# DecaYale/RNNPose

Hardware: AMD Instinct MI355X
Metric: pose-refine iters/sec (640x480, B=8, 3x8 recurrent) (higher is better)
Workload: dtype f32 (convolutions and volume build: fp16x3-split MFMA, fp32-class accuracy; LM: f64)

## Files before the change

rnnpose_amd/csrc/nhwc_ops.hip:

```cpp
#define RP_CONTRACT_LOCAL 1
#include "common.hpp"
#include "f16x3.cuh"
#include "induced.cuh"

namespace {

__global__ __launch_bounds__(256) void nchw_to_nhwc_kernel(const float* __restrict__ src, float* __restrict__ dst, int C,
                                                           int HW, int dst_cs, int dst_co) {
  __shared__ float tile[32][33];
  const int b = blockIdx.z;
  const int p0 = blockIdx.x * 32, c0 = blockIdx.y * 32;
  const int tx = threadIdx.x & 31, ty = threadIdx.x >> 5;
#pragma unroll
  for (int r = 0; r < 4; ++r) {
    const int c = c0 + ty + 8 * r, pp = p0 + tx;
    tile[ty + 8 * r][tx] = (c < C && pp < HW) ? src[(static_cast<long long>(b) * C + c) * HW + pp] : 0.f;
  }
  __syncthreads();
#pragma unroll
  for (int r = 0; r < 4; ++r) {
    const int pp = p0 + ty + 8 * r, c = c0 + tx;
    if (c < C && pp < HW) dst[(static_cast<long long>(b) * HW + pp) * dst_cs + dst_co + c] = tile[tx][ty + 8 * r];
  }
}

__global__ __launch_bounds__(256) void nhwc_to_nchw_kernel(const float* __restrict__ src, float* __restrict__ dst, int C,
                                                           int HW, int src_cs, int src_co) {
  __shared__ float tile[32][33];
  const int b = blockIdx.z;
  const int p0 = blockIdx.x * 32, c0 = blockIdx.y * 32;
  const int tx = threadIdx.x & 31, ty = threadIdx.x >> 5;
#pragma unroll
  for (int r = 0; r < 4; ++r) {
    const int pp = p0 + ty + 8 * r, c = c0 + tx;
    tile[ty + 8 * r][tx] = (c < C && pp < HW) ? src[(static_cast<long long>(b) * HW + pp) * src_cs + src_co + c] : 0.f;
  }
  __syncthreads();
#pragma unroll
  for (int r = 0; r < 4; ++r) {
    const int c = c0 + ty + 8 * r, pp = p0 + tx;
    if (c < C && pp < HW) dst[(static_cast<long long>(b) * C + c) * HW + pp] = tile[tx][ty + 8 * r];
  }
}

__global__ __launch_bounds__(256) void flow_prep_kernel(const float* __restrict__ coords1, float* __restrict__ flow4,
                                                        float* __restrict__ motion, int motion_cs, int motion_co, int h,
                                                        int w, long long total, int subtract_grid) {
  const long long t = static_cast<long long>(blockIdx.x) * blockDim.x + threadIdx.x;
  if (t >= total) return;
  const int n = h * w;
  const int b = static_cast<int>(t / n), pix = static_cast<int>(t - static_cast<long long>(b) * n);
  const int X = pix % w, Y = pix / w;
  const float fx = coords1[(static_cast<long long>(b) * 2 + 0) * n + pix] - (subtract_grid ? static_cast<float>(X) : 0.f);
  const float fy = coords1[(static_cast<long long>(b) * 2 + 1) * n + pix] - (subtract_grid ? static_cast<float>(Y) : 0.f);
  *reinterpret_cast<float4*>(flow4 + t * 4) = make_float4(fx, fy, 0.f, 0.f);
  *reinterpret_cast<float2*>(motion + t * motion_cs + motion_co) = make_float2(fx, fy);
}

__global__ __launch_bounds__(256) void conv3x3_cout2_kernel(const float* __restrict__ x, int cs, int co, int Cin,
                                                            const float* __restrict__ wgt, const float* __restrict__ bias,
                                                            const float* __restrict__ coords1, float* __restrict__ delta,
                                                            float* __restrict__ coords1_out, float* __restrict__ flow_lr,
                                                            int B, int h, int w) {
  extern __shared__ float wl[];
  const int tid = threadIdx.x;
  for (int e = tid; e < 2 * 9 * Cin; e += 256) {
    const int c = e % Cin, tap = (e / Cin) % 9, o = e / (9 * Cin);
    wl[e] = wgt[(static_cast<long long>(o) * Cin + c) * 9 + tap];
  }
  __syncthreads();
  const int lane = tid & 63, wave = tid >> 6;
  const int n = h * w;
  const long long total = static_cast<long long>(B) * n;
  for (long long p = static_cast<long long>(blockIdx.x) * 4 + wave; p < total; p += static_cast<long long>(gridDim.x) * 4) {
    const int b = static_cast<int>(p / n), pix = static_cast<int>(p - static_cast<long long>(b) * n);
    const int X = pix % w, Y = pix / w;
    float a0 = 0.f, a1 = 0.f;
    for (int c = lane * 4; c < Cin; c += 256) {
#pragma unroll
      for (int tap = 0; tap < 9; ++tap) {
        const int yy = Y + tap / 3 - 1, xx = X + tap % 3 - 1;
        if (yy < 0 || yy >= h || xx < 0 || xx >= w) continue;
        const float4 v = *reinterpret_cast<const float4*>(x + (static_cast<long long>(b) * n + yy * w + xx) * cs + co + c);
        const float4 w0 = *reinterpret_cast<const float4*>(wl + (0 * 9 + tap) * Cin + c);
        const float4 w1 = *reinterpret_cast<const float4*>(wl + (1 * 9 + tap) * Cin + c);
        a0 += v.x * w0.x + v.y * w0.y + v.z * w0.z + v.w * w0.w;
        a1 += v.x * w1.x + v.y * w1.y + v.z * w1.z + v.w * w1.w;
      }
    }
#pragma unroll
    for (int d = 32; d >= 1; d >>= 1) {
      a0 += __shfl_down(a0, d);
      a1 += __shfl_down(a1, d);
    }
    if (lane == 0) {
      const float dx = a0 + bias[0], dy = a1 + bias[1];
      *reinterpret_cast<float2*>(delta + p * 2) = make_float2(dx, dy);
      const float cx = coords1[(static_cast<long long>(b) * 2 + 0) * n + pix] + dx;
      const float cy = coords1[(static_cast<long long>(b) * 2 + 1) * n + pix] + dy;
      if (coords1_out) {
        coords1_out[(static_cast<long long>(b) * 2 + 0) * n + pix] = cx;
        coords1_out[(static_cast<long long>(b) * 2 + 1) * n + pix] = cy;
      }
      *reinterpret_cast<float2*>(flow_lr + p * 2) = make_float2(cx - static_cast<float>(X), cy - static_cast<float>(Y));
    }
  }
}

__global__ __launch_bounds__(256) void conv3x3_cout2_run4_kernel(const float* __restrict__ x, int cs, int co, int Cin,
                                                                 const float* __restrict__ wgt, const float* __restrict__ bias,
                                                                 const float* __restrict__ coords1, float* __restrict__ delta,
                                                                 float* __restrict__ coords1_out, float* __restrict__ flow_lr,
                                                                 int B, int h, int w) {
  const int lane = threadIdx.x & 63, wave = threadIdx.x >> 6;
  const int c = lane * 4;
  const bool cl = c < Cin;
  float4 w0[9], w1[9];
  {
    float t0[36], t1[36];
#pragma unroll
    for (int e = 0; e < 9; ++e) {
      const float4 z = make_float4(0.f, 0.f, 0.f, 0.f);
      const float4 q0 = cl ? *reinterpret_cast<const float4*>(wgt + (static_cast<long long>(0) * Cin + c) * 9 + e * 4) : z;
      const float4 q1 = cl ? *reinterpret_cast<const float4*>(wgt + (static_cast<long long>(1) * Cin + c) * 9 + e * 4) : z;
      t0[e * 4 + 0] = q0.x; t0[e * 4 + 1] = q0.y; t0[e * 4 + 2] = q0.z; t0[e * 4 + 3] = q0.w;
      t1[e * 4 + 0] = q1.x; t1[e * 4 + 1] = q1.y; t1[e * 4 + 2] = q1.z; t1[e * 4 + 3] = q1.w;
    }
#pragma unroll
    for (int tap = 0; tap < 9; ++tap) {
      w0[tap] = make_float4(t0[tap], t0[9 + tap], t0[18 + tap], t0[27 + tap]);
      w1[tap] = make_float4(t1[tap], t1[9 + tap], t1[18 + tap], t1[27 + tap]);
    }
  }
  const int n = h * w;
  const int runs_per_row = (w + 3) >> 2;
  const long long total_runs = static_cast<long long>(B) * h * runs_per_row;
  for (long long r = static_cast<long long>(blockIdx.x) * 4 + wave; r < total_runs; r += static_cast<long long>(gridDim.x) * 4) {
    const unsigned ru = static_cast<unsigned>(r);
    const unsigned by = ru / static_cast<unsigned>(runs_per_row);
    const int xr = static_cast<int>(ru - by * runs_per_row);
    const int b = static_cast<int>(by / static_cast<unsigned>(h)), Y = static_cast<int>(by - static_cast<unsigned>(b) * h);
    const int X0 = xr * 4;
    const int idx = ((lane >> 5) & 1) * 4 + ((lane >> 4) & 1) * 2 + ((lane >> 3) & 1);
    const int px = idx >> 1, o = idx & 1;
    const int Xw = X0 + px < w ? X0 + px : w - 1;
    const int pixw = Y * w + Xw;
    const float c1x = coords1[(static_cast<long long>(b) * 2 + 0) * n + pixw];
    const float c1y = coords1[(static_cast<long long>(b) * 2 + 1) * n + pixw];
    float4 v[3][6];
#pragma unroll
    for (int ry = 0; ry < 3; ++ry)
#pragma unroll
      for (int cx = 0; cx < 6; ++cx) {
        const int yy = Y + ry - 1, xx = X0 + cx - 1;
        const bool ok = cl && yy >= 0 && yy < h && xx >= 0 && xx < w;
        v[ry][cx] = ok ? *reinterpret_cast<const float4*>(x + (static_cast<long long>(b) * n + yy * w + xx) * cs + co + c)
                       : make_float4(0.f, 0.f, 0.f, 0.f);
      }
    float acc[8];
#pragma unroll
    for (int px = 0; px < 4; ++px) {
      float a0 = 0.f, a1 = 0.f;
#pragma unroll
      for (int ry = 0; ry < 3; ++ry)
#pragma unroll
        for (int k = 0; k < 3; ++k) {
          const float4 q = v[ry][px + k], u0 = w0[ry * 3 + k], u1 = w1[ry * 3 + k];
          a0 += q.x * u0.x + q.y * u0.y + q.z * u0.z + q.w * u0.w;
          a1 += q.x * u1.x + q.y * u1.y + q.z * u1.z + q.w * u1.w;
        }
      acc[px * 2 + 0] = a0;
      acc[px * 2 + 1] = a1;
    }
    float s4[4], s2[2], s1;
    {
      const bool up = lane & 32;
#pragma unroll
      for (int i = 0; i < 4; ++i) {
        const float keep = up ? acc[4 + i] : acc[i], give = up ? acc[i] : acc[4 + i];
        s4[i] = keep + __shfl_xor(give, 32);
      }
      const bool up2 = lane & 16;
#pragma unroll
      for (int i = 0; i < 2; ++i) {
        const float keep = up2 ? s4[2 + i] : s4[i], give = up2 ? s4[i] : s4[2 + i];
        s2[i] = keep + __shfl_xor(give, 16);
      }
      const bool up3 = lane & 8;
      const float keep = up3 ? s2[1] : s2[0], give = up3 ? s2[0] : s2[1];
      s1 = keep + __shfl_xor(give, 8);
      s1 += __shfl_xor(s1, 4);
      s1 += __shfl_xor(s1, 2);
      s1 += __shfl_xor(s1, 1);
    }
    const float other = __shfl_xor(s1, 8);
    if ((lane & 7) == 0 && o == 0 && X0 + px < w) {
      const int X = X0 + px, pix = Y * w + X;
      const long long p = static_cast<long long>(b) * n + pix;
      const float dx = s1 + bias[0], dy = other + bias[1];
      *reinterpret_cast<float2*>(delta + p * 2) = make_float2(dx, dy);
      const float cxv = c1x + dx;
      const float cyv = c1y + dy;
      if (coords1_out) {
        coords1_out[(static_cast<long long>(b) * 2 + 0) * n + pix] = cxv;
        coords1_out[(static_cast<long long>(b) * 2 + 1) * n + pix] = cyv;
      }
      *reinterpret_cast<float2*>(flow_lr + p * 2) = make_float2(cxv - static_cast<float>(X), cyv - static_cast<float>(Y));
    }
  }
}

__global__ __launch_bounds__(256) void convex_upsample_nhwc_kernel(const float* __restrict__ flow,
                                                                   const float* __restrict__ mask,
                                                                   float* __restrict__ up, int h, int w) {
  const int b = blockIdx.z, Y = blockIdx.y;
  const int X = blockIdx.x * 4 + (threadIdx.x >> 6);
  const int t = threadIdx.x & 63;
  if (X >= w) return;
  const int n = h * w;
  const float* m = mask + (static_cast<long long>(b) * n + Y * w + X) * 576 + t;
  float mv[9], mx = -INFINITY;
  float2 fv[9];
#pragma unroll
  for (int k = 0; k < 9; ++k) {
    mv[k] = m[k * 64];
    const int yy = Y + k / 3 - 1, xx = X + k % 3 - 1;
    const bool ok = yy >= 0 && yy < h && xx >= 0 && xx < w;
    fv[k] = *reinterpret_cast<const float2*>(flow + (static_cast<long long>(b) * n + (ok ? yy * w + xx : Y * w + X)) * 2);
  }
  __builtin_amdgcn_sched_barrier(0);
#pragma unroll
  for (int k = 0; k < 9; ++k) mx = fmaxf(mx, mv[k]);
  float den = 0.f;
#pragma unroll
  for (int k = 0; k < 9; ++k) {
    mv[k] = expf(mv[k] - mx);
    den += mv[k];
  }
  float ax = 0.f, ay = 0.f;
#pragma unroll
  for (int k = 0; k < 9; ++k) {
    const int yy = Y + k / 3 - 1, xx = X + k % 3 - 1;
    const float2 f = (yy >= 0 && yy < h && xx >= 0 && xx < w) ? fv[k] : make_float2(0.f, 0.f);
    const float wk = mv[k] / den;
    ax += wk * (8.f * f.x);
    ay += wk * (8.f * f.y);
  }
  const int i = t >> 3, j = t & 7;
  const long long Wf = 8LL * w, Pf = 64LL * n;
  const long long o = (8LL * Y + i) * Wf + 8 * X + j;
  up[(static_cast<long long>(b) * 2 + 0) * Pf + o] = ax;
  up[(static_cast<long long>(b) * 2 + 1) * Pf + o] = ay;
}


constexpr int IN_ROWS = 512;
__global__ __launch_bounds__(256) void instnorm_partial_kernel(const float* __restrict__ x, double* __restrict__ part,
                                                               int HW, int C) {
  __shared__ double s1[256], s2[256];
  const int b = blockIdx.y, chunk = blockIdx.x, nchunk = gridDim.x;
  const int tid = threadIdx.x;
  const int lanes_per_row = C >> 2;
  const int rows_per_iter = 256 / lanes_per_row;
  const int c4 = tid % lanes_per_row, r0 = tid / lanes_per_row;
  const int row_beg = chunk * IN_ROWS, row_end = min(HW, row_beg + IN_ROWS);
  double a[4] = {0, 0, 0, 0}, q[4] = {0, 0, 0, 0};
  if (r0 < rows_per_iter) {
    for (int r = row_beg + r0; r < row_end; r += rows_per_iter) {
      const float4 v = *reinterpret_cast<const float4*>(x + (static_cast<long long>(b) * HW + r) * C + c4 * 4);
      a[0] += v.x; a[1] += v.y; a[2] += v.z; a[3] += v.w;
      q[0] += static_cast<double>(v.x) * v.x; q[1] += static_cast<double>(v.y) * v.y;
      q[2] += static_cast<double>(v.z) * v.z; q[3] += static_cast<double>(v.w) * v.w;
    }
  }
  for (int k = 0; k < 4; ++k) {
    s1[tid] = a[k];
    s2[tid] = q[k];
    __syncthreads();
    if (tid < lanes_per_row) {
      double t1 = 0, t2 = 0;
      for (int g = 0; g < rows_per_iter; ++g) {
        t1 += s1[g * lanes_per_row + tid];
        t2 += s2[g * lanes_per_row + tid];
      }
      const int c = tid * 4 + k;
      part[((static_cast<long long>(b) * nchunk + chunk) * C + c) * 2 + 0] = t1;
      part[((static_cast<long long>(b) * nchunk + chunk) * C + c) * 2 + 1] = t2;
    }
    __syncthreads();
  }
}

__global__ void instnorm_finalize_kernel(const double* __restrict__ part, float* __restrict__ mean_rstd, int nchunk, int C,
                                         int HW, float eps) {
  const int b = blockIdx.x;
  for (int c = threadIdx.x; c < C; c += blockDim.x) {
    double t1 = 0, t2 = 0;
    for (int k = 0; k < nchunk; ++k) {
      t1 += part[((static_cast<long long>(b) * nchunk + k) * C + c) * 2 + 0];
      t2 += part[((static_cast<long long>(b) * nchunk + k) * C + c) * 2 + 1];
    }
    const double m = t1 / HW;
    double var = t2 / HW - m * m;
    if (var < 0) var = 0;
    mean_rstd[(static_cast<long long>(b) * C + c) * 2 + 0] = static_cast<float>(m);
    mean_rstd[(static_cast<long long>(b) * C + c) * 2 + 1] = static_cast<float>(1.0 / sqrt(var + static_cast<double>(eps)));
  }
}

__global__ __launch_bounds__(256) void instnorm_finalize_tiles_kernel(const double* __restrict__ tile_stats,
                                                                      float* __restrict__ mean_rstd, int tiles_per_image,
                                                                      int C, int HW, float eps) {
  __shared__ double s1[32][8], s2[32][8];
  const int b = blockIdx.x, cl = threadIdx.x & 7, c = blockIdx.y * 8 + cl, g = threadIdx.x >> 3;
  double t1 = 0, t2 = 0;
  if (c < C) {
    const double* p = tile_stats + (static_cast<long long>(b) * tiles_per_image * C + c) * 2;
#pragma unroll 4
    for (int k = g; k < tiles_per_image; k += 32) {
      const double2 v = *reinterpret_cast<const double2*>(p + static_cast<long long>(k) * C * 2);
      t1 += v.x;
      t2 += v.y;
    }
  }
  s1[g][cl] = t1;
  s2[g][cl] = t2;
  __syncthreads();
  if (g == 0 && c < C) {
    double a1 = 0, a2 = 0;
    for (int k = 0; k < 32; ++k) { a1 += s1[k][cl]; a2 += s2[k][cl]; }
    const double m = a1 / HW;
    double var = a2 / HW - m * m;
    if (var < 0) var = 0;
    mean_rstd[(static_cast<long long>(b) * C + c) * 2 + 0] = static_cast<float>(m);
    mean_rstd[(static_cast<long long>(b) * C + c) * 2 + 1] = static_cast<float>(1.0 / sqrt(var + static_cast<double>(eps)));
  }
}

__global__ __launch_bounds__(256) void instnorm_apply_kernel(const float* __restrict__ x, const float* __restrict__ mean_rstd,
                                                             const float* __restrict__ residual, float* __restrict__ out,
                                                             int HW, int C, int relu, long long total4,
                                                             const float* __restrict__ res_mr, int res_relu) {
  const long long i = static_cast<long long>(blockIdx.x) * blockDim.x + threadIdx.x;
  if (i >= total4) return;
  const unsigned iu = static_cast<unsigned>(i), cq = static_cast<unsigned>(C >> 2);
  const unsigned row = iu / cq;
  const int c4 = static_cast<int>(iu - row * cq);
  const int b = static_cast<int>(row / static_cast<unsigned>(HW));
  const float4 v = reinterpret_cast<const float4*>(x)[i];
  const float4 m01 = *reinterpret_cast<const float4*>(mean_rstd + (static_cast<long long>(b) * C + c4 * 4) * 2);
  const float4 m23 = *reinterpret_cast<const float4*>(mean_rstd + (static_cast<long long>(b) * C + c4 * 4 + 2) * 2);
  const float* rsrc = residual ? residual : x;
  const float* qsrc = res_mr ? res_mr : mean_rstd;
  float4 r = reinterpret_cast<const float4*>(rsrc)[i];
  const float4 q01 = *reinterpret_cast<const float4*>(qsrc + (static_cast<long long>(b) * C + c4 * 4) * 2);
  const float4 q23 = *reinterpret_cast<const float4*>(qsrc + (static_cast<long long>(b) * C + c4 * 4 + 2) * 2);
  __builtin_amdgcn_sched_barrier(0);
  float4 y = make_float4((v.x - m01.x) * m01.y, (v.y - m01.z) * m01.w, (v.z - m23.x) * m23.y, (v.w - m23.z) * m23.w);
  if (relu) y = make_float4(fmaxf(y.x, 0.f), fmaxf(y.y, 0.f), fmaxf(y.z, 0.f), fmaxf(y.w, 0.f));
  if (residual) {
    if (res_mr) {
      r = make_float4((r.x - q01.x) * q01.y, (r.y - q01.z) * q01.w, (r.z - q23.x) * q23.y, (r.w - q23.z) * q23.w);
      if (res_relu) r = make_float4(fmaxf(r.x, 0.f), fmaxf(r.y, 0.f), fmaxf(r.z, 0.f), fmaxf(r.w, 0.f));
// ... 194 lines not shown
    }
  }
  float4 r;
  r.x = ly0 * (lx0 * v[0].x + lx1 * v[1].x) + ly1 * (lx0 * v[2].x + lx1 * v[3].x);
  r.y = ly0 * (lx0 * v[0].y + lx1 * v[1].y) + ly1 * (lx0 * v[2].y + lx1 * v[3].y);
  r.z = ly0 * (lx0 * v[0].z + lx1 * v[1].z) + ly1 * (lx0 * v[2].z + lx1 * v[3].z);
  r.w = ly0 * (lx0 * v[0].w + lx1 * v[1].w) + ly1 * (lx0 * v[2].w + lx1 * v[3].w);
  *reinterpret_cast<float4*>(dst + static_cast<long long>(m) * dcs + dco + c) = r;
}

constexpr int PH_PIX = 64, PH_CH = 64, PH_CIN = 256, PH_COUT = 32;

__global__ __launch_bounds__(256) void pixel_head_nhwc_kernel(const float* __restrict__ src, int scs, int sco, int c_in,
                                                              const float* __restrict__ mean_rstd, int relu,
                                                              const float* __restrict__ wgt, const float* __restrict__ bias,
                                                              int c_out, int mode, float* __restrict__ dst, int HW, int npix) {
  __shared__ float w_s[PH_CIN * PH_COUT];
  __shared__ float x_s[PH_PIX * (PH_CH + 1)];
  __shared__ float ss_s[4 * PH_PIX];
  const int tid = threadIdx.x, lane = tid & 63, g = tid >> 6;
  for (int e = tid; e < PH_CIN * PH_COUT; e += 256) {
    const int c = e / PH_COUT, o = e % PH_COUT;
    w_s[e] = (c < c_in && o < c_out) ? wgt[o * c_in + c] : 0.f;
  }
  const bool active = g * 8 < c_out;
  float bo[8];
#pragma unroll
  for (int j = 0; j < 8; ++j) bo[j] = (g * 8 + j < c_out) ? bias[g * 8 + j] : 0.f;
  __syncthreads();
  const int ntiles = (npix + PH_PIX - 1) / PH_PIX;
  for (int tile = blockIdx.x; tile < ntiles; tile += gridDim.x) {
    const int n0 = tile * PH_PIX;
    float acc[8];
#pragma unroll
    for (int j = 0; j < 8; ++j) acc[j] = bo[j];
    for (int c0 = 0; c0 < c_in; c0 += PH_CH) {
      __syncthreads();
#pragma unroll
      for (int i = 0; i < 4; ++i) {
        const int e = tid + 256 * i, p = e >> 4, c = c0 + 4 * (e & 15);
        const int n = n0 + p;
        float4 v = make_float4(0.f, 0.f, 0.f, 0.f);
        if (n < npix && c < c_in) {
          v = *reinterpret_cast<const float4*>(src + static_cast<long long>(n) * scs + sco + c);
          if (mean_rstd) {
            const float* ms = mean_rstd + (static_cast<long long>(n / HW) * c_in + c) * 2;
            v.x = (v.x - ms[0]) * ms[1];
            v.y = (v.y - ms[2]) * ms[3];
            v.z = (v.z - ms[4]) * ms[5];
            v.w = (v.w - ms[6]) * ms[7];
          }
          if (relu) {
            v.x = fmaxf(v.x, 0.f);
            v.y = fmaxf(v.y, 0.f);
            v.z = fmaxf(v.z, 0.f);
            v.w = fmaxf(v.w, 0.f);
          }
        }
        float* xp = x_s + p * (PH_CH + 1) + 4 * (e & 15);
        xp[0] = v.x;
        xp[1] = v.y;
        xp[2] = v.z;
        xp[3] = v.w;
      }
      __syncthreads();
      if (active) {
        const int cn = c_in - c0 < PH_CH ? c_in - c0 : PH_CH;
        const float* xr = x_s + lane * (PH_CH + 1);
        for (int c = 0; c < cn; ++c) {
          const float x = xr[c];
          const float4 wa = *reinterpret_cast<const float4*>(w_s + (c0 + c) * PH_COUT + g * 8);
          const float4 wb = *reinterpret_cast<const float4*>(w_s + (c0 + c) * PH_COUT + g * 8 + 4);
          acc[0] = fmaf(x, wa.x, acc[0]);
          acc[1] = fmaf(x, wa.y, acc[1]);
          acc[2] = fmaf(x, wa.z, acc[2]);
          acc[3] = fmaf(x, wa.w, acc[3]);
          acc[4] = fmaf(x, wb.x, acc[4]);
          acc[5] = fmaf(x, wb.y, acc[5]);
          acc[6] = fmaf(x, wb.z, acc[6]);
          acc[7] = fmaf(x, wb.w, acc[7]);
        }
      }
    }
    float scale = 1.f;
    if (mode == 1) {
      float ss = 0.f;
#pragma unroll
      for (int j = 0; j < 8; ++j) ss = fmaf(acc[j], acc[j], ss);
      ss_s[g * PH_PIX + lane] = active ? ss : 0.f;
      __syncthreads();
      const float tot = (ss_s[lane] + ss_s[PH_PIX + lane]) + (ss_s[2 * PH_PIX + lane] + ss_s[3 * PH_PIX + lane]);
      scale = 1.f / fmaxf(sqrtf(tot), 1e-12f);
    }
    const int n = n0 + lane;
    if (active && n < npix) {
      const int b = n / HW, pix = n - b * HW;
      float* o = dst + (static_cast<long long>(b) * c_out + g * 8) * HW + pix;
#pragma unroll
      for (int j = 0; j < 8; ++j) {
        if (g * 8 + j >= c_out) break;
        float y = acc[j];
        if (mode == 1) y = acc[j] * scale;
        else if (mode == 2) y = 1.f / (1.f + expf(-y));
        o[static_cast<long long>(j) * HW] = y;
      }
    }
  }
}

}

extern "C" {

int rnnpose_nchw_to_nhwc_f32(const float* src, int B, int C, int HW, float* dst, int dst_c_stride, int dst_c_offset,
                             rnnpose_stream_t stream) {
  const char* fn = "rnnpose_nchw_to_nhwc_f32";
  RP_REQUIRE(src && dst, fn, "null pointer");
  RP_REQUIRE(B > 0 && B < 65536 && C > 0 && HW > 0 && dst_c_offset >= 0 && dst_c_offset + C <= dst_c_stride, fn, "bad size");
  hipLaunchKernelGGL(nchw_to_nhwc_kernel, dim3(rp::cdiv(HW, 32), rp::cdiv(C, 32), B), dim3(256), 0, rp::as_stream(stream),
                     src, dst, C, HW, dst_c_stride, dst_c_offset);
  return rp::check_launch(fn);
}

int rnnpose_nhwc_to_nchw_f32(const float* src, int B, int C, int HW, int src_c_stride, int src_c_offset, float* dst,
                             rnnpose_stream_t stream) {
  const char* fn = "rnnpose_nhwc_to_nchw_f32";
  RP_REQUIRE(src && dst, fn, "null pointer");
  RP_REQUIRE(B > 0 && B < 65536 && C > 0 && HW > 0 && src_c_offset >= 0 && src_c_offset + C <= src_c_stride, fn, "bad size");
  hipLaunchKernelGGL(nhwc_to_nchw_kernel, dim3(rp::cdiv(HW, 32), rp::cdiv(C, 32), B), dim3(256), 0, rp::as_stream(stream),
                     src, dst, C, HW, src_c_stride, src_c_offset);
  return rp::check_launch(fn);
}

int rnnpose_flow_prep_f32(const float* coords1, int subtract_grid, int B, int h, int w, float* flow4, float* motion,
                          int motion_c_stride, int motion_c_offset, rnnpose_stream_t stream) {
  const char* fn = "rnnpose_flow_prep_f32";
  RP_REQUIRE(coords1 && flow4 && motion, fn, "null pointer");
  RP_REQUIRE(B > 0 && h > 0 && w > 0 && motion_c_offset % 2 == 0 && motion_c_stride % 2 == 0 &&
                 motion_c_offset + 2 <= motion_c_stride, fn, "bad size");
  const long long total = static_cast<long long>(B) * h * w;
  hipLaunchKernelGGL(flow_prep_kernel, dim3(rp::cdiv(total, 256)), dim3(256), 0, rp::as_stream(stream), coords1, flow4,
                     motion, motion_c_stride, motion_c_offset, h, w, total, subtract_grid);
  return rp::check_launch(fn);
}

int rnnpose_flow_head_out_f32(const float* x, int x_c_stride, int x_c_offset, int c_in, const float* w_oihw,
                              const float* bias, const float* coords1, int B, int h, int w, float* delta,
                              float* coords1_out, float* flow_lr, rnnpose_stream_t stream) {
  const char* fn = "rnnpose_flow_head_out_f32";
  RP_REQUIRE(x && w_oihw && bias && coords1 && delta && flow_lr, fn, "null pointer");
  RP_REQUIRE(B > 0 && h > 0 && w > 0 && c_in > 0 && c_in % 4 == 0 && c_in <= 1024, fn, "bad size");
  RP_REQUIRE(x_c_stride % 4 == 0 && x_c_offset % 4 == 0 && x_c_offset + c_in <= x_c_stride, fn, "bad channel window");
  RP_REQUIRE(reinterpret_cast<uintptr_t>(w_oihw) % 16 == 0 && reinterpret_cast<uintptr_t>(x) % 16 == 0, fn, "x and weights must be 16-byte aligned");
  const long long total = static_cast<long long>(B) * h * w;
  if (c_in <= 256) {
    const long long runs = static_cast<long long>(B) * h * ((w + 3) / 4);
    RP_REQUIRE(runs < (1LL << 31), fn, "too many pixel runs for 32-bit indices");
#ifndef RP_COUT2_MAXWG
#define RP_COUT2_MAXWG 512
#endif
    const int nb = static_cast<int>(runs / 4 + 1 < RP_COUT2_MAXWG ? runs / 4 + 1 : RP_COUT2_MAXWG);
    hipLaunchKernelGGL(conv3x3_cout2_run4_kernel, dim3(nb), dim3(256), 0, rp::as_stream(stream), x, x_c_stride, x_c_offset, c_in,
                       w_oihw, bias, coords1, delta, coords1_out, flow_lr, B, h, w);
    return rp::check_launch(fn);
  }
  const int blocks = static_cast<int>(total / 4 + 1 < 4096 ? total / 4 + 1 : 4096);
  const size_t lds = static_cast<size_t>(2) * 9 * c_in * sizeof(float);
  hipLaunchKernelGGL(conv3x3_cout2_kernel, dim3(blocks), dim3(256), lds, rp::as_stream(stream), x, x_c_stride, x_c_offset,
                     c_in, w_oihw, bias, coords1, delta, coords1_out, flow_lr, B, h, w);
  return rp::check_launch(fn);
}

int rnnpose_convex_upsample_nhwc_f32(const float* flow_lr, const float* mask, int B, int h, int w, float* flow_up,
                                     rnnpose_stream_t stream) {
  const char* fn = "rnnpose_convex_upsample_nhwc_f32";
  RP_REQUIRE(flow_lr && mask && flow_up, fn, "null pointer");
  RP_REQUIRE(B > 0 && B < 65536 && h > 0 && h < 65536 && w > 0, fn, "bad size");
  hipLaunchKernelGGL(convex_upsample_nhwc_kernel, dim3(rp::cdiv(w, 4), h, B), dim3(256), 0, rp::as_stream(stream), flow_lr,
                     mask, flow_up, h, w);
  return rp::check_launch(fn);
}


size_t rnnpose_instnorm_workspace_bytes(int B, int HW, int C) {
  if (B <= 0 || HW <= 0 || C <= 0) return 0;
  return static_cast<size_t>(B) * rp::cdiv(HW, IN_ROWS) * C * 2 * sizeof(double);
}

int rnnpose_instnorm_nhwc_f32(const float* x, int B, int HW, int C, float eps, int relu, const float* residual,
                              void* workspace, size_t workspace_bytes, float* mean_rstd, float* out,
                              rnnpose_stream_t stream) {
  const char* fn = "rnnpose_instnorm_nhwc_f32";
  RP_REQUIRE(x && workspace && mean_rstd && out, fn, "null pointer");
  RP_REQUIRE(B > 0 && B < 65536 && HW > 0 && C >= 32 && C <= 256 && 1024 % C == 0 || C == 96 || C == 192, fn,
             "C must be 32, 64, 96, 128, 192 or 256");
  RP_REQUIRE(workspace_bytes >= rnnpose_instnorm_workspace_bytes(B, HW, C), fn, "workspace too small");
  const int nchunk = rp::cdiv(HW, IN_ROWS);
  hipStream_t st = rp::as_stream(stream);
  hipLaunchKernelGGL(instnorm_partial_kernel, dim3(nchunk, B), dim3(256), 0, st, x, static_cast<double*>(workspace), HW, C);
  hipLaunchKernelGGL(instnorm_finalize_kernel, dim3(B), dim3(256), 0, st, static_cast<const double*>(workspace), mean_rstd,
                     nchunk, C, HW, eps);
  const long long total4 = static_cast<long long>(B) * HW * (C >> 2);
  RP_REQUIRE(total4 < (1LL << 31), fn, "tensor too large for 32-bit float4 indices");
  hipLaunchKernelGGL(instnorm_apply_kernel, dim3(rp::cdiv(total4, 256)), dim3(256), 0, st, x, mean_rstd, residual, out, HW,
                     C, relu, total4, static_cast<const float*>(nullptr), 0);
  return rp::check_launch(fn);
}


int rnnpose_instnorm_tiles_nhwc_f32(const float* x, int B, int HW, int C, float eps, int relu, const float* residual,
                                    const float* residual_mean_rstd, int residual_relu, const double* tile_stats,
                                    int tiles_per_image, float* mean_rstd, float* out, rnnpose_stream_t stream) {
  const char* fn = "rnnpose_instnorm_tiles_nhwc_f32";
  RP_REQUIRE(tile_stats && mean_rstd && (x || !out), fn, "null pointer");
  RP_REQUIRE(B > 0 && B < 65536 && HW > 0 && C > 0 && C % 4 == 0, fn, "bad size (C % 4 == 0)");
  RP_REQUIRE(tiles_per_image > 0, fn, "tiles_per_image must be positive");
  hipStream_t st = rp::as_stream(stream);
  hipLaunchKernelGGL(instnorm_finalize_tiles_kernel, dim3(B, rp::cdiv(C, 8)), dim3(256), 0, st, tile_stats, mean_rstd, tiles_per_image, C, HW, eps);
  if (out) {
    const long long total4 = static_cast<long long>(B) * HW * (C >> 2);
    RP_REQUIRE(total4 < (1LL << 31), fn, "tensor too large for 32-bit float4 indices");
    hipLaunchKernelGGL(instnorm_apply_kernel, dim3(rp::cdiv(total4, 256)), dim3(256), 0, st, x, mean_rstd, residual, out, HW,
                       C, relu, total4, residual ? residual_mean_rstd : nullptr, residual_relu);
  }
  return rp::check_launch(fn);
}

int rnnpose_flow_conv7x7_relu_f32(const float* flow4, const float* w_t, const float* bias, int B, int h, int w, int c_out,
                                  float* out, int out_c_stride, int out_c_offset, rnnpose_stream_t stream) {
  const char* fn = "rnnpose_flow_conv7x7_relu_f32";
  RP_REQUIRE(flow4 && w_t && bias && out, fn, "null pointer");
  RP_REQUIRE(B > 0 && B < 65536 && h > 0 && h < 65536 && w > 0 && c_out > 0 && c_out <= 128, fn, "bad size (c_out <= 128)");
  RP_REQUIRE(out_c_offset >= 0 && out_c_offset + c_out <= out_c_stride && reinterpret_cast<uintptr_t>(flow4) % 16 == 0, fn,
             "bad output window / flow4 alignment");
  hipLaunchKernelGGL(conv7x7_cin2_kernel<false>, dim3(rp::cdiv(w, F1_TX), h, B), dim3(128), 0, rp::as_stream(stream), flow4, w_t,
                     bias, out, out_c_stride, out_c_offset, c_out, h, w, 0, static_cast<float*>(nullptr), 0, 0, 0, 0, 1.f,
                     static_cast<unsigned long long*>(nullptr), rp::InducedSrc{});
  return rp::check_launch(fn);
}

static int launch_flow_features(const char* fn, const float* coords1, const rp::InducedSrc isrc, int subtract_grid, const float* w_t, const float* bias,
                                int B, int h, int w, int c_out, float* out, int out_c_stride, int out_c_offset, float* motion, int motion_c_stride,
                                int motion_c_offset, int out_split, int motion_split, float a_scale, rnnpose_stream_t stream) {
  if (out_split) RP_REQUIRE(c_out % 2 == 0 && out_c_offset % 8 == 0 && out_c_stride % 8 == 0 && reinterpret_cast<uintptr_t>(out) % 32 == 0 && a_scale > 0.f, fn,
                            "split-form out: even c_out, channel offset/stride multiples of 8, 32-byte aligned");
  if (motion_split) RP_REQUIRE(motion_c_stride % 8 == 0 && reinterpret_cast<uintptr_t>(motion) % 32 == 0 && a_scale > 0.f, fn,
                               "split-form motion: channel stride multiple of 8, 32-byte aligned");
  RP_REQUIRE((coords1 || isrc.depth) && w_t && bias && out && motion, fn, "null pointer");
  RP_REQUIRE(B > 0 && B < 65536 && h > 0 && h < 65536 && w > 0 && c_out > 0 && c_out <= 128, fn, "bad size (c_out <= 128)");
  RP_REQUIRE(out_c_offset >= 0 && out_c_offset + c_out <= out_c_stride && motion_c_offset % 2 == 0 && motion_c_stride % 2 == 0 &&
                 motion_c_offset + 2 <= motion_c_stride, fn, "bad output windows");
  hipLaunchKernelGGL(conv7x7_cin2_kernel<true>, dim3(rp::cdiv(w, F1_TX), h, B), dim3(128), 0, rp::as_stream(stream), coords1, w_t,
                     bias, out, out_c_stride, out_c_offset, c_out, h, w, subtract_grid, motion, motion_c_stride, motion_c_offset,
                     out_split, motion_split, a_scale, rp::sat_counter(), isrc);
  return rp::check_launch(fn);
}

int rnnpose_flow_features_f32(const float* coords1, int subtract_grid, const float* w_t, const float* bias, int B, int h, int w,
                              int c_out, float* out, int out_c_stride, int out_c_offset, float* motion, int motion_c_stride,
                              int motion_c_offset, int out_split, int motion_split, float a_scale, rnnpose_stream_t stream) {
  return launch_flow_features("rnnpose_flow_features_f32", coords1, rp::InducedSrc{}, subtract_grid, w_t, bias, B, h, w, c_out, out, out_c_stride,
                              out_c_offset, motion, motion_c_stride, motion_c_offset, out_split, motion_split, a_scale, stream);
}

int rnnpose_flow_features_induced_f32(const float* depth, const float* K, const float* G, int H, int W, float eps, const float* w_t,
                                      const float* bias, int B, int h, int w, int c_out, float* out, int out_c_stride, int out_c_offset,
                                      float* motion, int motion_c_stride, int motion_c_offset, int out_split, int motion_split, float a_scale,
                                      rnnpose_stream_t stream) {
  const char* fn = "rnnpose_flow_features_induced_f32";
  RP_REQUIRE(depth && K && G && H >= h && W >= w && W / (w > 0 ? w : 1) >= 1, fn, "null pointer / the depth map must be at least as large as the low-resolution map");
  return launch_flow_features(fn, nullptr, rp::InducedSrc{depth, K, G, H, W, eps}, 1, w_t, bias, B, h, w, c_out, out, out_c_stride, out_c_offset, motion,
                              motion_c_stride, motion_c_offset, out_split, motion_split, a_scale, stream);
}

int rnnpose_split_hl_f32(const float* src, int src_c_stride, int src_c_offset, long long n_pixels, int c_count, float a_scale,
                         float* dst, int dst_c_stride, int dst_c_offset, rnnpose_stream_t stream) {
  const char* fn = "rnnpose_split_hl_f32";
  RP_REQUIRE(src && dst && n_pixels > 0 && c_count > 0 && a_scale > 0.f, fn, "bad argument");
  RP_REQUIRE(c_count % 8 == 0 && src_c_offset % 4 == 0 && src_c_stride % 4 == 0 && dst_c_offset % 8 == 0 && dst_c_stride % 8 == 0 &&
                 src_c_offset + c_count <= src_c_stride && dst_c_offset + c_count <= dst_c_stride &&
                 reinterpret_cast<uintptr_t>(src) % 16 == 0 && reinterpret_cast<uintptr_t>(dst) % 32 == 0, fn,
             "whole 8-channel groups, aligned channel windows");
  const long long total = n_pixels * (c_count / 8);
  hipLaunchKernelGGL(split_hl_kernel, dim3(rp::cdiv(total, 256)), dim3(256), 0, rp::as_stream(stream), src, src_c_stride, src_c_offset,
                     dst, dst_c_stride, dst_c_offset, c_count / 8, total, a_scale, rp::sat_counter());
  return rp::check_launch(fn);
}

static bool quad_window(const float* p, int c_stride, int c_offset, int c) {
  return c > 0 && c % 4 == 0 && c_offset >= 0 && c_offset % 4 == 0 && c_stride % 4 == 0 && c_offset + c <= c_stride &&
         reinterpret_cast<uintptr_t>(p) % 16 == 0;
}

int rnnpose_maxpool2x2_nhwc_f32(const float* src, int B, int H, int W, int src_c_stride, int src_c_offset, int C, float* dst,
                                int dst_c_stride, int dst_c_offset, rnnpose_stream_t stream) {
  const char* fn = "rnnpose_maxpool2x2_nhwc_f32";
  RP_REQUIRE(src && dst, fn, "null pointer");
  RP_REQUIRE(B > 0 && H >= 2 && W >= 2, fn, "bad size (H, W >= 2)");
  RP_REQUIRE(static_cast<long long>(B) * H * W < (1LL << 31), fn, "B * H * W must be below 2^31");
  RP_REQUIRE(quad_window(src, src_c_stride, src_c_offset, C) && quad_window(dst, dst_c_stride, dst_c_offset, C), fn,
             "channel windows: C, offsets and strides multiples of 4, inside the stride, 16-byte aligned tensors");
  const int Ho = H / 2, Wo = W / 2;
  const long long total = static_cast<long long>(B) * Ho * Wo * (C / 4);
  hipLaunchKernelGGL(maxpool2x2_nhwc_kernel, dim3(rp::cdiv(total, 256)), dim3(256), 0, rp::as_stream(stream), src, src_c_stride,
                     src_c_offset, dst, dst_c_stride, dst_c_offset, H, W, Ho, Wo, C / 4, total);
  return rp::check_launch(fn);
}

int rnnpose_upsample2x_bilinear_nhwc_f32(const float* src, int B, int h, int w, int src_c_stride, int src_c_offset, int C,
                                         const float* mean_rstd, int relu, float* dst, int dst_c_stride, int dst_c_offset,
                                         rnnpose_stream_t stream) {
  const char* fn = "rnnpose_upsample2x_bilinear_nhwc_f32";
  RP_REQUIRE(src && dst, fn, "null pointer");
  RP_REQUIRE(B > 0 && h > 0 && w > 0, fn, "bad size");
  RP_REQUIRE(static_cast<long long>(B) * h * w * 4 < (1LL << 31), fn, "B * 2h * 2w must be below 2^31");
  RP_REQUIRE(quad_window(src, src_c_stride, src_c_offset, C) && quad_window(dst, dst_c_stride, dst_c_offset, C), fn,
             "channel windows: C, offsets and strides multiples of 4, inside the stride, 16-byte aligned tensors");
  RP_REQUIRE(!mean_rstd || reinterpret_cast<uintptr_t>(mean_rstd) % 16 == 0, fn, "mean_rstd must be 16-byte aligned");
// ... 525 lines not shown
```

Before: 786.4.

## Compute flow-head 3x3 Cout=2 conv with fp32 MFMA over 2D halo tiles

Replaces the per-row-run shuffle-reduction kernel for the flow head's 3x3 conv with 2 outputs by a tiled kernel. Each block loads a 7x18 halo of a 5x16 pixel tile and multiplies it against an 18-column weight matrix (9 taps x 2 outputs) using fp32 32x32x2 MFMA. Partial products go to LDS, and the epilogue sums the 9 shifted taps per pixel. It also remaps block IDs across XCDs and launches one block per tile. The cost is about 60% recompute on halo pixels and more LDS traffic, in exchange for moving the dot products onto matrix cores.

```diff
diff --git a/rnnpose_amd/csrc/nhwc_ops.hip b/rnnpose_amd/csrc/nhwc_ops.hip
--- a/rnnpose_amd/csrc/nhwc_ops.hip
+++ b/rnnpose_amd/csrc/nhwc_ops.hip
@@ -107,108 +107,112 @@
   }
 }
 
-__global__ __launch_bounds__(256) void conv3x3_cout2_run4_kernel(const float* __restrict__ x, int cs, int co, int Cin,
+constexpr int kPH = 5, kPW = 16;
+constexpr int kHW = kPW + 2;
+constexpr int kHalo = (kPH + 2) * kHW;
+constexpr int kN = 18;
+constexpr int kMaxCin = 256;
+static_assert(kHalo <= 128 && kPH * kPW * 2 <= 256, "four 32-row tiles, one epilogue thread per (pixel, output)");
+
+__global__ __launch_bounds__(256, 2) void flow_head_tiles_kernel(const float* __restrict__ x, int cs, int co, int Cin,
                                                                  const float* __restrict__ wgt, const float* __restrict__ bias,
-                                                                 const float* __restrict__ coords1, float* __restrict__ delta,
-                                                                 float* __restrict__ coords1_out, float* __restrict__ flow_lr,
-                                                                 int B, int h, int w) {
-  const int lane = threadIdx.x & 63, wave = threadIdx.x >> 6;
-  const int c = lane * 4;
-  const bool cl = c < Cin;
-  float4 w0[9], w1[9];
+                                                                 const float* coords1, float* __restrict__ delta,
+                                                                 float* coords1_out, float* __restrict__ flow_lr, int h, int w,
+                                                                 int tiles_x, int tiles_per_image) {
+  __shared__ float4 wl[kMaxCin / 4 * kN];
+  __shared__ float pl[128 * kN];
+  const int tid = threadIdx.x, lane = tid & 63, wave = tid >> 6;
+  int bid = blockIdx.x;
   {
-    float t0[36], t1[36];
-#pragma unroll
-    for (int e = 0; e < 9; ++e) {
-      const float4 z = make_float4(0.f, 0.f, 0.f, 0.f);
-      const float4 q0 = cl ? *reinterpret_cast<const float4*>(wgt + (static_cast<long long>(0) * Cin + c) * 9 + e * 4) : z;
-      const float4 q1 = cl ? *reinterpret_cast<const float4*>(wgt + (static_cast<long long>(1) * Cin + c) * 9 + e * 4) : z;
-      t0[e * 4 + 0] = q0.x; t0[e * 4 + 1] = q0.y; t0[e * 4 + 2] = q0.z; t0[e * 4 + 3] = q0.w;
-      t1[e * 4 + 0] = q1.x; t1[e * 4 + 1] = q1.y; t1[e * 4 + 2] = q1.z; t1[e * 4 + 3] = q1.w;
-    }
-#pragma unroll
-    for (int tap = 0; tap < 9; ++tap) {
-      w0[tap] = make_float4(t0[tap], t0[9 + tap], t0[18 + tap], t0[27 + tap]);
-      w1[tap] = make_float4(t1[tap], t1[9 + tap], t1[18 + tap], t1[27 + tap]);
-    }
-  }
-  const int n = h * w;
-  const int runs_per_row = (w + 3) >> 2;
-  const long long total_runs = static_cast<long long>(B) * h * runs_per_row;
-  for (long long r = static_cast<long long>(blockIdx.x) * 4 + wave; r < total_runs; r += static_cast<long long>(gridDim.x) * 4) {
-    const unsigned ru = static_cast<unsigned>(r);
-    const unsigned by = ru / static_cast<unsigned>(runs_per_row);
-    const int xr = static_cast<int>(ru - by * runs_per_row);
-    const int b = static_cast<int>(by / static_cast<unsigned>(h)), Y = static_cast<int>(by - static_cast<unsigned>(b) * h);
-    const int X0 = xr * 4;
-    const int idx = ((lane >> 5) & 1) * 4 + ((lane >> 4) & 1) * 2 + ((lane >> 3) & 1);
-    const int px = idx >> 1, o = idx & 1;
-    const int Xw = X0 + px < w ? X0 + px : w - 1;
-    const int pixw = Y * w + Xw;
-    const float c1x = coords1[(static_cast<long long>(b) * 2 + 0) * n + pixw];
-    const float c1y = coords1[(static_cast<long long>(b) * 2 + 1) * n + pixw];
-    float4 v[3][6];
-#pragma unroll
-    for (int ry = 0; ry < 3; ++ry)
-#pragma unroll
-      for (int cx = 0; cx < 6; ++cx) {
-        const int yy = Y + ry - 1, xx = X0 + cx - 1;
-        const bool ok = cl && yy >= 0 && yy < h && xx >= 0 && xx < w;
-        v[ry][cx] = ok ? *reinterpret_cast<const float4*>(x + (static_cast<long long>(b) * n + yy * w + xx) * cs + co + c)
-                       : make_float4(0.f, 0.f, 0.f, 0.f);
-      }
-    float acc[8];
-#pragma unroll
-    for (int px = 0; px < 4; ++px) {
-      float a0 = 0.f, a1 = 0.f;
-#pragma unroll
-      for (int ry = 0; ry < 3; ++ry)
-#pragma unroll
-        for (int k = 0; k < 3; ++k) {
-          const float4 q = v[ry][px + k], u0 = w0[ry * 3 + k], u1 = w1[ry * 3 + k];
-          a0 += q.x * u0.x + q.y * u0.y + q.z * u0.z + q.w * u0.w;
-          a1 += q.x * u1.x + q.y * u1.y + q.z * u1.z + q.w * u1.w;
-        }
-      acc[px * 2 + 0] = a0;
-      acc[px * 2 + 1] = a1;
-    }
-    float s4[4], s2[2], s1;
-    {
-      const bool up = lane & 32;
-#pragma unroll
-      for (int i = 0; i < 4; ++i) {
-        const float keep = up ? acc[4 + i] : acc[i], give = up ? acc[i] : acc[4 + i];
-        s4[i] = keep + __shfl_xor(give, 32);
-      }
-      const bool up2 = lane & 16;
-#pragma unroll
-      for (int i = 0; i < 2; ++i) {
-        const float keep = up2 ? s4[2 + i] : s4[i], give = up2 ? s4[i] : s4[2 + i];
-        s2[i] = keep + __shfl_xor(give, 16);
-      }
-      const bool up3 = lane & 8;
-      const float keep = up3 ? s2[1] : s2[0], give = up3 ? s2[0] : s2[1];
-      s1 = keep + __shfl_xor(give, 8);
-      s1 += __shfl_xor(s1, 4);
-      s1 += __shfl_xor(s1, 2);
-      s1 += __shfl_xor(s1, 1);
-    }
-    const float other = __shfl_xor(s1, 8);
-    if ((lane & 7) == 0 && o == 0 && X0 + px < w) {
-      const int X = X0 + px, pix = Y * w + X;
-      const long long p = static_cast<long long>(b) * n + pix;
-      const float dx = s1 + bias[0], dy = other + bias[1];
-      *reinterpret_cast<float2*>(delta + p * 2) = make_float2(dx, dy);
-      const float cxv = c1x + dx;
-      const float cyv = c1y + dy;
-      if (coords1_out) {
-        coords1_out[(static_cast<long long>(b) * 2 + 0) * n + pix] = cxv;
-        coords1_out[(static_cast<long long>(b) * 2 + 1) * n + pix] = cyv;
-      }
-      *reinterpret_cast<float2*>(flow_lr + p * 2) = make_float2(cxv - static_cast<float>(X), cyv - static_cast<float>(Y));
-    }
-  }
-}
+    const int per = gridDim.x >> 3, rem = gridDim.x & 7;
+    const int xcd = bid & 7, idx = bid >> 3;
+    bid = xcd * per + (xcd < rem ? xcd : rem) + idx;
+  }
+  const int b = bid / tiles_per_image, t = bid - b * tiles_per_image;
+  const int ty = t / tiles_x, y0 = ty * kPH, x0 = (t - ty * tiles_x) * kPW;
+  const int n = h * w, nj = Cin >> 3;
+  const long long img = static_cast<long long>(b) * n;
+
+  const int nq = kN * Cin / 4;
+  float4 wq[5];
+#pragma unroll
+  for (int i = 0; i < 5; ++i) {
+    const int q = tid + 256 * i;
+    wq[i] = reinterpret_cast<const float4*>(wgt)[q < nq ? q : nq - 1];
+  }
+  __builtin_amdgcn_s_barrier();
+  const int hh = lane >> 5, m = wave * 32 + (lane & 31);
+  const int hy = m / kHW, hx = m - hy * kHW;
+  const int Ya = y0 - 1 + hy, Xa = x0 - 1 + hx;
+  const bool a_ok = m < kHalo && Ya >= 0 && Ya < h && Xa >= 0 && Xa < w;
+  const float* src = x + (img + (a_ok ? Ya * w + Xa : y0 * w + x0)) * cs + co + 4 * hh;
+  float4 a[kMaxCin / 8];
+#pragma unroll
+  for (int j = 0; j < kMaxCin / 8; ++j) a[j] = *reinterpret_cast<const float4*>(src + 8 * (j < nj ? j : 0));
+  const int eo = tid & 1, epix = tid >> 1;
+  const int ely = epix / kPW, elx = epix - ely * kPW;
+  const int Ye = y0 + ely, Xe = x0 + elx;
+  const bool e_ok = tid < kPH * kPW * 2 && Ye < h && Xe < w;
+  const int pe = e_ok ? Ye * w + Xe : y0 * w + x0;
+  const float c1 = coords1[(img * 2 + static_cast<long long>(eo) * n) + pe];
+  const float bo = bias[eo];
+  __builtin_amdgcn_sched_barrier(0);
+
+  float* wlf = reinterpret_cast<float*>(wl);
+#pragma unroll
+  for (int i = 0; i < 5; ++i) {
+    const int q = tid + 256 * i < nq ? tid + 256 * i : nq - 1;
+    const float v[4] = {wq[i].x, wq[i].y, wq[i].z, wq[i].w};
+#pragma unroll
+    for (int u = 0; u < 4; ++u) {
+      const int f = 4 * q + u;
+      const int o = f >= Cin * 9, rem = f - o * Cin * 9;
+      const int c = rem / 9, tap = rem - 9 * c;
+      wlf[((c >> 2) * kN + tap * 2 + o) * 4 + (c & 3)] = v[u];
+    }
+  }
+  __syncthreads();
+
+  const int col = lane & 31;
+  const bool col_ok = col < kN;
+  const float4 z4 = make_float4(0.f, 0.f, 0.f, 0.f);
+  rp::f32x16 acc, acc1;
+#pragma unroll
+  for (int i = 0; i < 16; ++i) acc[i] = acc1[i] = 0.f;
+#pragma unroll
+  for (int j = 0; j < kMaxCin / 8; ++j) {
+    const float4 bq = wl[(2 * (j < nj ? j : 0) + hh) * kN + (col_ok ? col : 0)];
+    const float4 bv = col_ok ? bq : z4;
+    const float4 av = a_ok && j < nj ? a[j] : z4;
+    acc = __builtin_amdgcn_mfma_f32_32x32x2f32(av.x, bv.x, acc, 0, 0, 0);
+    acc1 = __builtin_amdgcn_mfma_f32_32x32x2f32(av.y, bv.y, acc1, 0, 0, 0);
+    acc = __builtin_amdgcn_mfma_f32_32x32x2f32(av.z, bv.z, acc, 0, 0, 0);
+    acc1 = __builtin_amdgcn_mfma_f32_32x32x2f32(av.w, bv.w, acc1, 0, 0, 0);
+  }
+#pragma unroll
+  for (int i = 0; i < 16; ++i) acc[i] += acc1[i];
+  if (col_ok) {
+#pragma unroll
+    for (int i = 0; i < 16; ++i) {
+      const int row = wave * 32 + (i & 3) + 8 * (i >> 2) + 4 * hh;
+      pl[row * kN + col] = acc[i];
+    }
+  }
+  __syncthreads();
+
+  if (e_ok) {
+    float s = 0.f;
+#pragma unroll
+    for (int tap = 0; tap < 9; ++tap) s += pl[((ely + tap / 3) * kHW + elx + tap % 3) * kN + tap * 2 + eo];
+    const float d = s + bo;
+    const float cv = c1 + d;
+    const long long p = img + pe;
+    delta[p * 2 + eo] = d;
+    if (coords1_out) coords1_out[(img * 2 + static_cast<long long>(eo) * n) + pe] = cv;
+    flow_lr[p * 2 + eo] = cv - static_cast<float>(eo ? Ye : Xe);
+  }
+}
+
 
 __global__ __launch_bounds__(256) void convex_upsample_nhwc_kernel(const float* __restrict__ flow,
                                                                    const float* __restrict__ mask,
@@ -709,18 +713,15 @@
   RP_REQUIRE(B > 0 && h > 0 && w > 0 && c_in > 0 && c_in % 4 == 0 && c_in <= 1024, fn, "bad size");
   RP_REQUIRE(x_c_stride % 4 == 0 && x_c_offset % 4 == 0 && x_c_offset + c_in <= x_c_stride, fn, "bad channel window");
   RP_REQUIRE(reinterpret_cast<uintptr_t>(w_oihw) % 16 == 0 && reinterpret_cast<uintptr_t>(x) % 16 == 0, fn, "x and weights must be 16-byte aligned");
+  if (c_in % 32 == 0 && c_in <= 256) {
+    const int tiles_x = rp::cdiv(w, kPW), tiles_per_image = tiles_x * rp::cdiv(h, kPH);
+    RP_REQUIRE(static_cast<long long>(h) * w < (1LL << 31) && static_cast<long long>(B) * tiles_per_image < (1LL << 31), fn,
+               "map too large for 32-bit indices");
+    hipLaunchKernelGGL(flow_head_tiles_kernel, dim3(B * tiles_per_image), dim3(256), 0, rp::as_stream(stream), x, x_c_stride,
+                       x_c_offset, c_in, w_oihw, bias, coords1, delta, coords1_out, flow_lr, h, w, tiles_x, tiles_per_image);
+    return rp::check_launch(fn);
+  }
   const long long total = static_cast<long long>(B) * h * w;
-  if (c_in <= 256) {
-    const long long runs = static_cast<long long>(B) * h * ((w + 3) / 4);
-    RP_REQUIRE(runs < (1LL << 31), fn, "too many pixel runs for 32-bit indices");
-#ifndef RP_COUT2_MAXWG
-#define RP_COUT2_MAXWG 512
-#endif
-    const int nb = static_cast<int>(runs / 4 + 1 < RP_COUT2_MAXWG ? runs / 4 + 1 : RP_COUT2_MAXWG);
-    hipLaunchKernelGGL(conv3x3_cout2_run4_kernel, dim3(nb), dim3(256), 0, rp::as_stream(stream), x, x_c_stride, x_c_offset, c_in,
-                       w_oihw, bias, coords1, delta, coords1_out, flow_lr, B, h, w);
-    return rp::check_launch(fn);
-  }
   const int blocks = static_cast<int>(total / 4 + 1 < 4096 ? total / 4 + 1 : 4096);
   const size_t lds = static_cast<size_t>(2) * 9 * c_in * sizeof(float);
   hipLaunchKernelGGL(conv3x3_cout2_kernel, dim3(blocks), dim3(256), lds, rp::as_stream(stream), x, x_c_stride, x_c_offset,
```

Result: no change. 786.1 (-0.0%).
